# CommonRoad/commonroad-reactive-planner

Measured on AMD Instinct MI355X. Metric: candidate trajectories/sec (sample+cost+collision) per replan, higher is better.
Workload: dtype f64; 1 GPU; cfg3: DEU_Test-1_1_T-1, 31x31x63 grid, N=60, 51 obstacles (49 synthetic, seed 0); mode=draw, horizon_steps=60, n_obstacles=51, parallelism=one GPU, exchange=none

## Files before the change

commonroad-reactive-planner_amd/csrc/rp_host.hip:

```cpp
#include <hip/hip_runtime.h>
#include <hip/hip_ext.h>
#include <sched.h>

#include <algorithm>
#include <atomic>
#include <chrono>
#include <cmath>
#include <cstdio>
#include <cstdlib>
#include <cstring>
#include <mutex>
#include <new>
#include <string>
#include <unordered_map>
#include <vector>

#include "rp_kernels.h"
#include "rp_frontend.h"
#include "rp_corridor.h"
#include "rp_pool.h"
#include "rp_fold_static.h"
#include "rp_table_window.h"

namespace {
// ... 6 lines not shown
constexpr int kChunkMinWavesPerCU = 7;
constexpr int kCostMinPerCU = 832;
constexpr int kSweepMinPerCU = 512;
constexpr int kLazyCap[RP_LAZY_LEVELS] = {1024, 4096, 16384};
constexpr int kLazyOff[RP_LAZY_LEVELS] = {0, 1024, 5120};
constexpr int kLazyListWords = 21504;
constexpr uint32_t kLazyTarget[RP_LAZY_LEVELS] = {128, 1024, 8192};

using ResultBlock = FinalizeOut;

struct Options {
    int lanes = 0;
    int eval_block = 0;
    int cost_kernel = -1;
    int chunk_kernel = -1;
    int lazy = -1;
    int sweep = -1;
    int fused_lon = 1;
    int fused_lon_blocks = -1;
    int auto_materialize = 1;
    int shard_policy = 1;
    int stage_out = 1, row_padding = 1, row_align = 0, tail_split = 1;
    int fixed_stride = 1;
    int table_window = 1;
    int lean_broad = 1;
    int fold_static = -1;
    int fold_threshold = kFoldThreshold;
    int lon_publish = 1, inline_grids = 1, event_bracket = 0, winner_lanes_as_batch = 0, zero_copy = 1, coeff_groups = 1;
    int winner_skip_query = 1;
    int lazy_trace = 0, print_stamps = 0, timing = 0;
    int wait_mode = RP_WAIT_SPIN;
};
struct OptionDesc {
    const char *key;
    int Options::*field;
    const char *env;
    bool env_negates;
    int lo, hi;
};
const OptionDesc kOptionTable[] = {
    {"lanes", &Options::lanes, "RP_AMD_G", false, 0, 64},
    {"eval_block", &Options::eval_block, "RP_AMD_EVAL_BLOCK", false, 0, 256},
    {"cost_kernel", &Options::cost_kernel, "RP_AMD_COST_KERNEL", false, -1, 1},
    {"chunk_kernel", &Options::chunk_kernel, "RP_AMD_CHUNK_KERNEL", false, -1, 1},
    {"lazy", &Options::lazy, "RP_AMD_LAZY", false, -1, 1},
    {"sweep", &Options::sweep, "RP_AMD_SWEEP", false, -1, 1},
    {"fused_lon", &Options::fused_lon, "RP_AMD_NO_FUSED_LON", true, 0, 1},
    {"fused_lon_blocks", &Options::fused_lon_blocks, "RP_AMD_FUSED_LON_BLOCKS", false, -1, 1 << 20},
    {"auto_materialize", &Options::auto_materialize, "RP_AMD_NO_AUTO_MATERIALIZE", true, 0, 1},
    {"shard_policy", &Options::shard_policy, "RP_AMD_SHARD_POLICY", false, 0, 1},
    {"stage_out", &Options::stage_out, "RP_AMD_NO_STAGE_OUT", true, 0, 1},
    {"row_padding", &Options::row_padding, "RP_AMD_NO_ROW_PADDING", true, 0, 1},
    {"row_align", &Options::row_align, "RP_AMD_ROW_ALIGN", false, 0, 16},
    {"tail_split", &Options::tail_split, "RP_AMD_NO_TAIL_SPLIT", true, 0, 1},
    {"fixed_stride", &Options::fixed_stride, "RP_AMD_NO_FIXED_STRIDE", true, 0, 1},
    {"table_window", &Options::table_window, "RP_AMD_NO_TABLE_WINDOW", true, 0, 1},
    {"lean_broad", &Options::lean_broad, "RP_AMD_NO_LEAN_BROAD", true, 0, 1},
    {"fold_static", &Options::fold_static, "RP_AMD_FOLD_STATIC", false, -1, 1},
    {"fold_threshold", &Options::fold_threshold, "RP_AMD_FOLD_THRESHOLD", false, 1, 1 << 30},
    {"lon_publish", &Options::lon_publish, "RP_AMD_NO_LON_PUBLISH", true, 0, 1},
    {"inline_grids", &Options::inline_grids, "RP_AMD_NO_INLINE_GRIDS", true, 0, 1},
    {"event_bracket", &Options::event_bracket, "RP_AMD_EVENT_BRACKET", false, 0, 1},
    {"winner_lanes_as_batch", &Options::winner_lanes_as_batch, "RP_AMD_WINNER_G_AS_BATCH", false, 0, 1},
    {"winner_skip_query", &Options::winner_skip_query, "RP_AMD_NO_WINNER_SKIP_QUERY", true, 0, 1},
    {"zero_copy", &Options::zero_copy, "RP_AMD_NO_ZERO_COPY", true, 0, 1},
    {"coeff_groups", &Options::coeff_groups, "RP_AMD_NO_COEFF_GROUPS", true, 0, 1},
    {"lazy_trace", &Options::lazy_trace, "RP_AMD_LAZY_TRACE", false, 0, 1},
    {"print_stamps", &Options::print_stamps, "RP_AMD_PRINT_STAMPS", false, 0, 1},
    {"timing", &Options::timing, "RP_AMD_TIMING", false, 0, 1},
    {"wait_mode", &Options::wait_mode, "RP_AMD_WAIT_MODE", false, RP_WAIT_SPIN, RP_WAIT_EVENT},
};
const OptionDesc *find_option(const char *key) {
    if (!key) return nullptr;
    for (const OptionDesc &d : kOptionTable)
        if (std::strcmp(d.key, key) == 0) return &d;
    return nullptr;
}
void options_from_environment(Options &o) {
    for (const OptionDesc &d : kOptionTable) {
        const char *e = d.env ? std::getenv(d.env) : nullptr;
        if (!e) continue;
        const int v = d.env_negates ? 0 : std::atoi(e);
        if (v >= d.lo && v <= d.hi) o.*(d.field) = v;
    }
}

}

struct rp_ctx {
    Options opt;
    int device = 0;
    hipStream_t stream = nullptr;
    std::string err;
    int num_cus = 256;
    int profiling = 0;
    unsigned long long calls = 0;
    hipEvent_t ev0 = nullptr, ev1 = nullptr;
    bool time_next_launch = false, timed_by_launch = false;

    double *d_tables = nullptr;
    int n_ref = 0, search_iters = 0, n_buckets = 0, table_words = 0;
    double bucket_inv_h = 0.0;
    double proj_d_limit = 20.0;
    std::vector<double> h_pos;
    rpfe::Tables h_front;
    std::vector<double> cycle_buf;
// ... 21 lines not shown
    double *d_states = nullptr;
    double *d_compact = nullptr;
    size_t cap_compact = 0;
    size_t cap_states = 0;
    double *d_profile = nullptr, *d_profile_one = nullptr;
    size_t cap_profile = 0, cap_profile_one = 0;
    PairHdr *d_pair_hdr = nullptr, *d_pair_hdr_one = nullptr;
    size_t cap_pair_hdr = 0;
    void *d_partials = nullptr;
    int cap_partials = 0;
    unsigned long long *d_sel_scratch = nullptr;
    LazyCtl *d_lazy_ctl = nullptr;
    int32_t *d_lazy_lists = nullptr;
    uint32_t *d_lazy_hist = nullptr;
    double *d_lazy_states = nullptr;
    size_t cap_lazy_states = 0;
    int lazy_skip = 0, lazy_penalty = 0;
    int collision_mode = RP_COLLISION_AUTO;
    int last_kernel = 0;
    int last_fixed_stride = 0;
#ifdef RP_TIMELINE_LON
    int last_lon_grid = 0;
#endif
    int last_lon_lean = 0;
    int last_collision_level = 0;
    int last_lazy = 0;
    double last_best_cost = 0.0;
    int64_t last_best_index = -1;
    double path_us[2] = {0.0, 0.0};
    int path_n[2] = {0, 0};
    int path_since_probe = 0, path_regime = -1;
    bool path_adaptive = false;
    bool time_whole = false;
    std::chrono::steady_clock::time_point plan_t0;
    bool epilogue_dirty = false;
    struct Pending {
        bool active = false, cin = false, skip_eval = false, ticket = false, done = false, time_valid = false, mat = false, coeffs = false;
        unsigned long long seq = 0;
        int grid = 0;
        KArgs ka{};
        std::chrono::steady_clock::time_point tp0, tp1;
    } pending;
    struct LevelState {
        Pending pending;
        std::vector<char> staged;
        bool staged_on_device = false, last_rows_on_device = false;
// ... 142 lines not shown
int collision_level(const KArgs &ka) {
    if (!ka.has_obstacles || (ka.flags & RP_FLAG_SKIP_COLLISION)) return 0;
    return (ka.obs.n_sobb + ka.obs.n_tri + ka.obs.n_circ) > 0 ? 2 : 1;
}

const void *sweep_kernel_fn(bool cin, int coll, bool one_chunk) {
    if (cin) {
        if (coll == 2) return one_chunk ? (const void *)rp_eval_kernel<16, false, true, 2, true, false, false, RP_BLOCK, true> : (const void *)rp_eval_kernel<16, false, true, 2, false, false, false, RP_BLOCK, true>;
        return one_chunk ? (const void *)rp_eval_kernel<16, false, true, 1, true, false, false, RP_BLOCK, true> : (const void *)rp_eval_kernel<16, false, true, 1, false, false, false, RP_BLOCK, true>;
    }
    if (coll == 2) return one_chunk ? (const void *)rp_eval_kernel<16, false, false, 2, true, false, false, RP_BLOCK, true> : (const void *)rp_eval_kernel<16, false, false, 2, false, false, false, RP_BLOCK, true>;
    return one_chunk ? (const void *)rp_eval_kernel<16, false, false, 1, true, false, false, RP_BLOCK, true> : (const void *)rp_eval_kernel<16, false, false, 1, false, false, false, RP_BLOCK, true>;
}

const void *chunk_kernel_fn(bool low, int coll) {
    if (low) return coll == 2 ? (const void *)rp_chunk_kernel<true, 2> : (coll == 1 ? (const void *)rp_chunk_kernel<true, 1> : (const void *)rp_chunk_kernel<true, 0>);
    return coll == 2 ? (const void *)rp_chunk_kernel<false, 2> : (coll == 1 ? (const void *)rp_chunk_kernel<false, 1> : (const void *)rp_chunk_kernel<false, 0>);
}

inline bool fixed_stride_applies(const rp_ctx *c, const KArgs &ka) {
    return ka.row_stride == RP_ROW64 && ka.tail_split == 0 && ka.N + 1 > 16 && ka.N + 1 <= RP_ROW64 && c->opt.fixed_stride != 0;
}

template <int G, bool MAT, bool CIN, int COLL, bool STAGE>
void launch_eval_tcs(rp_ctx *c, const KArgs &ka, int grid, size_t lds, int block = RP_BLOCK) {
    if constexpr (G == 16 && MAT && !STAGE) {
        if (fixed_stride_applies(c, ka)) {
            if (block == 64) launch_kargs(c, (const void *)rp_eval_kernel<G, MAT, CIN, COLL, false, false, false, 64, false, true>, grid, 64, lds, ka);
            else launch_kargs(c, (const void *)rp_eval_kernel<G, MAT, CIN, COLL, false, false, false, RP_BLOCK, false, true>, grid, RP_BLOCK, lds, ka);
            return;
        }
    }
    if constexpr (G == 16 && !STAGE) {
        if (block == 64) {
            if (ka.N + 1 <= G) launch_kargs(c, (const void *)rp_eval_kernel<G, MAT, CIN, COLL, true, false, false, 64>, grid, 64, lds, ka);
            else launch_kargs(c, (const void *)rp_eval_kernel<G, MAT, CIN, COLL, false, false, false, 64>, grid, 64, lds, ka);
            return;
        }
    }
    if (ka.N + 1 <= G) launch_kargs(c, (const void *)rp_eval_kernel<G, MAT, CIN, COLL, true, STAGE, false>, grid, RP_BLOCK, lds, ka);
    else launch_kargs(c, (const void *)rp_eval_kernel<G, MAT, CIN, COLL, false, STAGE, false>, grid, RP_BLOCK, lds, ka);
}

constexpr int kFusedLonG = 16;
constexpr size_t kFusedLonLdsLimit = 61440;
int fused_lon_max_blocks(const rp_ctx *c) {
    if (c->opt.fused_lon_blocks >= 0) return c->opt.fused_lon_blocks;
    return c->num_cus * 4;
}

// ... 469 lines not shown
        const bool cost_rows_ok = (unsigned long long)ka.pair_count * PF_FIELDS * (unsigned long long)(ka.N + 1) * 8ull < (1ull << 32);
        const bool cost_big = count >= (int64_t)c->num_cus * 1024;
        auto lane_kernel_for = [&](int coll) -> int {
            if (!lane_kernel_ok) return 0;
            if (c->opt.chunk_kernel == 1 && chunk_G) return 2;
            if (!cost_rows_ok) return (chunk_G && c->opt.chunk_kernel != 0 && coll == 0) ? 2 : 0;
            if (c->opt.cost_kernel == 1) return 1;
            if (coll > 0) return (c->opt.cost_kernel != 0 && cost_big) ? 1 : 0;
            const int64_t chunk_waves = ((count + RP_CHUNK_BLOCK - 1) / RP_CHUNK_BLOCK) * chunk_G;
            const bool chunk_ok = c->opt.chunk_kernel != 0 && chunk_G && chunk_G <= 4 && chunk_waves >= (int64_t)c->num_cus * kChunkMinWavesPerCU;
            if (c->opt.cost_kernel != 0 && count >= (int64_t)c->num_cus * (chunk_ok ? kCostMinPerCU : (ka.N + 1 <= 64 ? 240 : 448))) return 1;
            return chunk_ok ? 2 : 0;
        };
        auto launch_main_eval = [&](const KArgs &k, bool mat_) -> int {
            c->timed_by_launch = false;
            c->time_next_launch = by_launch;
            if (timed && !by_launch) HIP_TRY(c, hipEventRecord(c->ev0, c->stream));
            const auto te0 = c->timing ? std::chrono::steady_clock::now() : std::chrono::steady_clock::time_point();
            const int coll = collision_level(k);
            const int which = mat_ ? 0 : lane_kernel_for(coll);
            if (which == 1) {
                main_grid = (int)((count + RP_COST_BLOCK - 1) / RP_COST_BLOCK);
                c->last_kernel = RP_KERNEL_COST;
                c->last_fixed_stride = 0;
                const void *fn = k.low_vel_mode
                    ? (coll == 2 ? (const void *)rp_cost_kernel<true, 2> : coll == 1 ? (const void *)rp_cost_kernel<true, 1> : (const void *)rp_cost_kernel<true, 0>)
                    : (coll == 2 ? (const void *)rp_cost_kernel<false, 2> : coll == 1 ? (const void *)rp_cost_kernel<false, 1> : (const void *)rp_cost_kernel<false, 0>);
                launch_kargs(c, fn, main_grid, RP_COST_BLOCK, 0, k);
            } else if (which == 2) {
                main_grid = (int)((count + RP_CHUNK_BLOCK - 1) / RP_CHUNK_BLOCK);
                c->last_kernel = RP_KERNEL_CHUNK;
                c->last_fixed_stride = 0;
                launch_kargs(c, chunk_kernel_fn(k.low_vel_mode != 0, coll), main_grid, RP_CHUNK_BLOCK * chunk_G, rp_chunk_lds_bytes(chunk_G), k);
            } else {
                main_grid = grid;
                c->last_kernel = RP_KERNEL_EVAL;
                c->last_fixed_stride = !fused_lds && mat_ && G == 16 && fixed_stride_applies(c, k);
                if (fused_lds) launch_eval_fused(c, k, grid, mat_, cin, fused_lds, G);
                else launch_eval(c, k, grid, mat_, cin, G, block);
            }
            if (c->timing) c->t_sum[4] += std::chrono::duration<double, std::micro>(std::chrono::steady_clock::now() - te0).count();
            c->time_next_launch = false;
            if (timed && !by_launch) HIP_TRY(c, hipEventRecord(c->ev1, c->stream));
            time_valid = timed && (!by_launch || c->timed_by_launch);
            return RP_OK;
        };
        bool lazy_possible = count > 0 && !mat && !fused_lds && collision_level(ka) > 0 && !(ka.flags & RP_FLAG_DRAW_ALL) &&
                             ka.cost_kind != RP_COST_EXTERNAL && !ka.single_index && !ka.gate;
        const int lazy_env = c->opt.lazy;
        lazy_possible = lazy_possible && lazy_env != 0 && (c->collision_mode != RP_COLLISION_EAGER || lazy_env == 1);
        const bool always = lazy_env == 1 || (lazy_env == -1 && c->collision_mode == RP_COLLISION_COST_ORDERED);
        bool lazy_try = lazy_possible && (always || (!small && c->lazy_skip == 0));
        if (lazy_possible && !lazy_try && !always && !small && c->lazy_skip > 0) --c->lazy_skip;
        c->path_adaptive = lazy_possible && lazy_env == -1 && !small && c->collision_mode == RP_COLLISION_TIMED;
        if (c->path_adaptive) {
            int lg = 0;
            while ((count >> (lg + 1)) != 0) ++lg;
            const int regime = 2 * lg + (cin ? 1 : 0);
            if (regime != c->path_regime) { c->path_regime = regime; c->path_n[0] = c->path_n[1] = 0; c->path_since_probe = 0; }
            if (lazy_try) {
// ... 335 lines not shown

int rp_last_path(const rp_ctx *c) { return c ? c->last_lazy : 0; }
int rp_last_kernel(const rp_ctx *c) { return c ? c->last_kernel : 0; }

int rp_set_collision_path(rp_ctx *c, int mode) {
    if (!c) return RP_EINVAL;
    if (mode < RP_COLLISION_AUTO || mode > RP_COLLISION_TIMED) return fail(c, RP_EINVAL, "rp_set_collision_path: unknown mode");
    if (mode != c->collision_mode) { c->lazy_skip = c->lazy_penalty = 0; c->path_regime = -1; }
    c->collision_mode = mode;
    return RP_OK;
}

int rp_set_profiling(rp_ctx *c, int enable) {
    if (!c) return RP_EINVAL;
    c->profiling = enable < 0 ? 0 : enable;
    return RP_OK;
}

int rp_set_option(rp_ctx *c, const char *key, int64_t value) {
    if (!c) return RP_EINVAL;
    if (c->pending.active) return fail(c, RP_ESTATE, "rp_set_option: a plan is in flight on this context (rp_plan_wait first)");
    const OptionDesc *d = find_option(key);
    if (!d) return fail(c, RP_EINVAL, std::string("rp_set_option: unknown option '") + (key ? key : "(null)") + "'");
    if (value < d->lo || value > d->hi) return fail(c, RP_EINVAL, std::string("rp_set_option: value out of range for '") + key + "'");
    c->opt.*(d->field) = (int)value;
    c->timing = c->opt.timing != 0;
    c->spin_wait = c->opt.wait_mode != RP_WAIT_EVENT;
    c->lazy_skip = c->lazy_penalty = 0; c->path_regime = -1;
    return RP_OK;
}

int rp_get_option(const rp_ctx *c, const char *key, int64_t *value) {
    if (!c || !value) return RP_EINVAL;
    if (key && std::strcmp(key, "wait_fallbacks") == 0) { *value = c->wait_fallbacks; return RP_OK; }
    if (key && std::strcmp(key, "last_fixed_stride") == 0) { *value = c->last_fixed_stride; return RP_OK; }
    if (key && std::strcmp(key, "last_lon_lean") == 0) { *value = c->last_lon_lean; return RP_OK; }
    if (key && std::strcmp(key, "last_collision_level") == 0) { *value = c->last_collision_level; return RP_OK; }
    if (key && std::strcmp(key, "fold_static_steps") == 0) { *value = c->d_fold ? c->fold_steps : 0; return RP_OK; }
    if (key && std::strcmp(key, "last_lanes") == 0) { *value = c->last_G; return RP_OK; }
    if (key && std::strcmp(key, "last_single_launch") == 0) { *value = c->last_fused_lds != 0 ? 1 : 0; return RP_OK; }
    if (key && std::strcmp(key, "last_table_window") == 0) { *value = c->have_last ? c->last.win_n : 0; return RP_OK; }
    if (key && std::strcmp(key, "last_table_window_first") == 0) { *value = c->have_last ? c->last.win_k0 : 0; return RP_OK; }
    const OptionDesc *d = find_option(key);
    if (!d) return RP_EINVAL;
    *value = c->opt.*(d->field);
    return RP_OK;
}

int rp_set_wait_mode(rp_ctx *c, int mode) { return rp_set_option(c, "wait_mode", mode); }
int rp_get_wait_mode(const rp_ctx *c) { return c ? c->opt.wait_mode : RP_WAIT_SPIN; }

int rp_set_reference(rp_ctx *c, int32_t n, const double *ref_pos, const double *ref_theta, const double *ref_curv,
                     const double *ref_curv_d, const double *ref_x, const double *ref_y, double proj_domain_d_limit) {
    if (!c) return RP_EINVAL;
    if (c->pending.active) return fail(c, RP_ESTATE, "rp_set_reference: a plan is in flight on this context (rp_plan_wait first)");
    if (n < 2 || !ref_pos || !ref_theta || !ref_curv || !ref_curv_d || !ref_x || !ref_y)
        return fail(c, RP_EINVAL, "rp_set_reference: need n >= 2 and six non-null tables");
    for (int i = 0; i + 1 < n; ++i)
// ... 1319 lines not shown
```

commonroad-reactive-planner_amd/csrc/rp_kernels.h:

```cpp
#pragma once

#include "rp_device.h"

#define RP_BLOCK 256
#ifndef RP_COPY_OUT_STORE
#define RP_COPY_OUT_STORE(p, v)                                                                                   \
    __builtin_nontemporal_store(*reinterpret_cast<const __attribute__((ext_vector_type(2))) double *>(&(v)),        \
                                reinterpret_cast<__attribute__((ext_vector_type(2))) double *>(p))
#endif
#ifndef RP_WAVES_PER_SIMD
#define RP_WAVES_PER_SIMD 3
#endif

struct KArgs {
    double dt;
    int32_t N, factor, time_step0, low_vel_mode, lon_mode;
    uint32_t constraint_mask, flags;
    double x0_lon[3], x0_lat[3], x0_orientation;
    double wheelbase, wb_rear_axle, half_length, half_width, ego_radius;
    double a_max, v_switch, v_delta_max, kappa_max;
    double c_yaw;
    double c_kdot;
    int32_t cost_kind, has_speed, has_s, partials_cap;
    double w_a, desired_speed, desired_d, desired_s;
// ... 899 lines not shown
    const bool fast = v > v_switch;
    const double acc_l = fast ? acc * v : acc, acc_r = fast ? a_max * v_switch : a_max;
    const bool bad_acc = !((-a_max <= acc) & (acc_l <= acc_r));
    const bool bad_v = v < -RP_EPS, bad_k = fabs(kappa) > kappa_max;
    reason = (((cm & RP_CHECK_ACCELERATION) != 0) & bad_acc) ? RP_REASON_ACCELERATION : reason;
    reason = (((cm & RP_CHECK_KAPPA_DOT) != 0) & bad_kd) ? RP_REASON_KAPPA_DOT : reason;
    reason = (((cm & RP_CHECK_YAW_RATE) != 0) & bad_yaw) ? RP_REASON_YAW_RATE : reason;
    reason = (((cm & RP_CHECK_KAPPA) != 0) & bad_k) ? RP_REASON_KAPPA : reason;
    reason = (((cm & RP_CHECK_VELOCITY) != 0) & bad_v) ? RP_REASON_VELOCITY : reason;
    return reason;
}

__device__ __forceinline__ void lateral_derivs(bool low, double dd, double ddd, double inv_sd, double sdd, double &dp, double &dpp) {
    if (!low) {
        dp = dd * inv_sd;
        const double ddot = ddd - dp * sdd;
        dpp = ddot * inv_sd * inv_sd;
    } else {
        dp = dd;
        dpp = ddd;
    }
}

__device__ __forceinline__ void atan_angles(double dp, double th_ref, double &th_cl, double &th_gl, double &cosT, double &secT, double &tanT) {
    th_cl = rp_atan(dp);
    th_gl = th_cl + th_ref;
    const double w2 = __builtin_fma(dp, dp, 1.0);
    cosT = rp_rsqrt(w2);
    secT = w2 * cosT;
    tanT = dp;
}

__device__ __forceinline__ void standstill_angles(double th_cl, bool use_atan, double &cosT, double &secT, double &tanT) {
    double sn, cs;
    rp_sincos(th_cl, &sn, &cs);
    const double sc = rp_rcp(cs);
    cosT = use_atan ? cosT : cs;
    secT = use_atan ? secT : sc;
    tanT = use_atan ? tanT : sn * sc;
}

__device__ __forceinline__ void frenet_kinematics(double d, double dp, double dpp, double sd, double sdd, double k_r, double k_r_d,
                                                  double cosT, double secT, double tanT, double &kappa, double &v, double &acc) {
    const double oneKrD = 1.0 - k_r * d;
    const double q = cosT * rp_rcp(oneKrD);
    const double kterm = frenet_kterm(k_r_d, d, k_r, dp);
    kappa = frenet_kappa(dpp, kterm, tanT, cosT, q, k_r);
    const double f = oneKrD * secT;
    v = sd * f;
    acc = frenet_acc(sdd, f, sd, secT, oneKrD, tanT, kappa, k_r, kterm);
}

__device__ __forceinline__ void extended_state(double l_v, double l_acc, double l_s, double l_sd, double l_d, double l_dd, double tk,
                                               double &vt, double &e_s, double &e_d) {
    vt = l_v + tk * l_acc;
    vt = vt * (vt >= 0.0 ? 1.0 : 0.0);
    e_s = l_s + tk * l_sd;
    e_d = l_d + tk * l_dd;
// ... 540 lines not shown
        pair = p32;
        ci.v[0] = grid_base(a)[a.nT + a.nL + (int)(g32 - p32 * nd)];
    }
    ci.pair_slot = pair - hdr_pair0;
}

__device__ __forceinline__ void fetch_header(const PairHdr *hdrs, CandIn &ci) {
    const PairHdr h = hdrs[ci.pair_slot];
    ci.lat_T = h.lat_T;
    ci.s0 = h.s0;
    ci.pre_reason = h.pre_reason;
    ci.L = h.L;
}

template <bool COEFFS_IN>
__device__ __forceinline__ CandIn fetch_candidate(const KArgs &a, int64_t gidx, const PairHdr *hdrs, int64_t hdr_pair0) {
    CandIn ci;
    fetch_lateral<COEFFS_IN>(a, gidx, ci, hdr_pair0);
    fetch_header(hdrs, ci);
    return ci;
}

#define RP_ROW64 64
template <int G, bool MAT, bool COEFFS_IN, int COLL, bool ONE_CHUNK, bool STAGE_OUT, bool LON_FUSED, int BLOCK = RP_BLOCK, bool SWEEP = false,
          bool ROW64 = false>
__global__ __launch_bounds__(BLOCK, RP_WAVES_PER_SIMD) void rp_eval_kernel(const KArgsG ag) {
    static_assert(!SWEEP || (G == 16 && !MAT && COLL != 0 && !STAGE_OUT && !LON_FUSED && BLOCK == RP_BLOCK), "the sweep's variant");
    static_assert(!ROW64 || (G == 16 && MAT && !ONE_CHUNK && !STAGE_OUT && !LON_FUSED && !SWEEP), "the fixed-stride variant");
    const KArgs &a = ag.k;
    extern __shared__ double lds_out[];
    static_assert(!(LON_FUSED && STAGE_OUT), "the single-launch variant stores state rows directly");
    constexpr bool RP_WT = LON_FUSED;
    constexpr bool RP_NT = MAT && !LON_FUSED && !STAGE_OUT;
    touch_kernargs<10>();

    const int tid = threadIdx.x;
    RP_STAMP(0);
    RP_TL(0);
    const int lane = tid & 63;
    const int gl = lane & (G - 1);
    const int gbase = lane & ~(G - 1);
    static_assert(BLOCK == RP_BLOCK || (!LON_FUSED && !STAGE_OUT), "smaller workgroups: plain two-kernel variants only");
    constexpr int GPB = BLOCK / G;
    constexpr int GPW = 64 / G;
    constexpr int PFN = COLL ? PF_FIELDS : PF_COS_REF;
    const int wave_in_block = tid >> 6;
    const int group_in_wave = gbase / G;
    const int grp = tid / G;

    if (level_gate_closed(a.gate, a.gate_seq, a.gate_level)) return;
    if (a.single_index && *a.single_index < 0) {
// ... 319 lines not shown
        if (al.has_s) { e = 0.25 * (al.desired_s - s); cst = __builtin_fma(e, e, cst); }
        if (i == N) {
            e = 20.0 * (al.desired_d - d); cst = __builtin_fma(e, e, cst);
            e = 5.0 * fabs(th_cl); cst = __builtin_fma(e, e, cst);
            if (al.has_speed) { e = v - al.desired_speed; cst += 50.0 * (e * e); }
            if (al.has_s) { e = 20.0 * (al.desired_s - s); cst = __builtin_fma(e, e, cst); }
        }
        if (i == mid && al.has_speed) { e = v - al.desired_speed; cst += 100.0 * (e * e); }
        return cst;
    };
    auto fetched_cost_terms = [&](const CostParams &cp, int i, double acc, double v, double s, double d, double th_cl) -> double {
        double e, cst;
        e = cp.w_a * acc; cst = e * e;
        e = 0.25 * (cp.desired_d - d); cst = __builtin_fma(e, e, cst);
        e = 0.25 * fabs(th_cl); cst = __builtin_fma(e, e, cst);
        if (cp.has_speed) { asm volatile(""); e = 5.0 * (v - cp.desired_speed); cst = __builtin_fma(e, e, cst); }
        if (cp.has_s) { asm volatile(""); e = 0.25 * (cp.desired_s - s); cst = __builtin_fma(e, e, cst); }
        if (i == N) {
            e = 20.0 * (cp.desired_d - d); cst = __builtin_fma(e, e, cst);
            e = 5.0 * fabs(th_cl); cst = __builtin_fma(e, e, cst);
            if (cp.has_speed) { asm volatile(""); e = v - cp.desired_speed; cst += 50.0 * (e * e); }
            if (cp.has_s) { asm volatile(""); e = 20.0 * (cp.desired_s - s); cst = __builtin_fma(e, e, cst); }
        }
        if (i == mid && cp.has_speed) { asm volatile(""); e = v - cp.desired_speed; cst += 100.0 * (e * e); }
        return cst;
    };

    if (wave_first < count) {
        const int64_t w0 = wave_first;
        const int64_t slot = w0 + group_in_wave;
        const bool valid = slot < count && sweep_need;
        const int64_t gidx = al.single_index ? *al.single_index
                             : ((!LON_FUSED && al.index_list) ? (int64_t)al.index_list[valid ? slot : w0] : al.cand_begin + (valid ? slot : w0));

        const int L = cin.L;
        const double s0 = cin.s0;
        const uint32_t pre_reason = (uint32_t)cin.pre_reason;
        const int32_t pair_slot_ = (int32_t)(pair_index<COEFFS_IN>(al, gidx) - pair0);
        const int32_t pair_w = __builtin_amdgcn_readfirstlane(pair_slot_);
        const uint32_t n8p = (uint32_t)n * 8u;
        const char *const pbase = reinterpret_cast<const char *>(prof_base + ((size_t)pair_w * PF_FIELDS) * (size_t)n);
        const uint32_t poff8 = (uint32_t)(pair_slot_ - pair_w) * PF_FIELDS * n8p;
        ProfStep pf = pf0;
        if (!LON_FUSED) {
            Poly lat;
            if (COEFFS_IN) lat = {cin.v[0], cin.v[1], cin.v[2], cin.v[3], cin.v[4], cin.v[5]};
            else lat = quintic_coeffs(al.x0_lat[0], al.x0_lat[1], al.x0_lat[2], cin.v[0], 0.0, 0.0, cin.lat_T);
// ... 53 lines not shown
                uint64_t near_sta_cell = 0;
                if (!SKIP_EXTENDED || __any(act)) {
                    const double t = (double)i * dt;
                    const double tau = low ? s - s0 : t;
                    d = poly_pos(gs_poly, tau); dd = poly_vel(gs_poly, tau); ddd = poly_acc(gs_poly, tau);
                    if (fabs(dd) < RP_EPS) dd = 0.0;
                    if (!LATE_STORE && store_ok && act) {
                        const uint32_t off8 = lane_off8 + (uint32_t)i * 8u;
                        st_row<RP_WT, RP_NT>(row_at(off8, RP_S), s);
                        st_row<RP_WT, RP_NT>(row_at(off8, RP_S_DOT), sd);
                        st_row<RP_WT, RP_NT>(row_at(off8, RP_S_DDOT), sdd);
                        st_row<RP_WT, RP_NT>(row_at(off8, RP_D), d);
                        st_row<RP_WT, RP_NT>(row_at(off8, RP_D_DOT), dd);
                        st_row<RP_WT, RP_NT>(row_at(off8, RP_D_DDOT), ddd);
                    }
                    RP_STAMP(3);

                    const bool moving = inv_sd > 0.0;
                    double dp, dpp;
                    lateral_derivs(low, dd, ddd, inv_sd, sdd, dp, dpp);

                    const bool use_atan = moving || low;
                    double cosT, secT, tanT;
                    atan_angles(dp, th_ref, th_cl, th_gl, cosT, secT, tanT);
                    if (__any(act && !use_atan)) {
                        const uint64_t mv = group_ballot<G>(use_atan && act, gbase);
                        const uint64_t below = mv & ((1ull << gl) - 1ull);
                        const int src = below ? 63 - __clzll(below) : 0;
                        const double th_from = group_bcast<G>(th_gl, src);
                        if (!use_atan) {
                            th_gl = below ? th_from : theta_carry;
                            th_cl = th_gl - th_ref;
                        }
                        standstill_angles(th_cl, use_atan, cosT, secT, tanT);
                    }
                    const double sinT = tanT * cosT;
                    cos_gl = heading_cos(pf.f[PF_COS_REF], pf.f[PF_SIN_REF], cosT, sinT);
                    sin_gl = heading_sin(pf.f[PF_COS_REF], pf.f[PF_SIN_REF], cosT, sinT);
                    RP_STAMP(5);

                    frenet_kinematics(d, dp, dpp, sd, sdd, k_r, k_r_d, cosT, secT, tanT, kappa, v, acc);

                    double th_prev = lane_prev(th_gl), ka_prev = lane_prev(kappa);
                    if (gl == 0) { th_prev = theta_carry; ka_prev = kappa_carry; }
                    const double dth = i > 0 ? th_gl - th_prev : 0.0;
                    kdot = i > 0 ? kappa - ka_prev : 0.0;
                    RP_STAMP(6);

                    uint32_t reason = constraint_reason(al, cm, v, acc, kappa, dth, kdot);
                    reason = act ? reason : RP_REASON_NONE;
                    if (__any(reason != RP_REASON_NONE)) {
                        const uint64_t fm = group_ballot<G>(reason != RP_REASON_NONE, gbase);
                        const int fl = fm ? __ffsll((unsigned long long)fm) - 1 : 0;
                        const uint32_t r_first = (uint32_t)__shfl((int)reason, fl, G);
                        if (fm && fail_step < 0) { fail_step = base + fl; fail_reason = r_first; }
                        if (!draw && fail_step >= 0) alive = false;
                        if (__ballot(alive) == 0) break;
                    }
                    RP_STAMP(7);

                    const bool in_dom = s_in_dom && fabs(d) <= al.proj_d_limit;
                    x = px + d * nx; y = py + d * ny;
                    if (__any(act && !in_dom) || ood_step >= 0) {
                        const uint64_t om = group_ballot<G>(act && !in_dom, gbase);
                        if (om && ood_step < 0) ood_step = base + __ffsll((unsigned long long)om) - 1;
                        if (ood_step >= 0 && i >= ood_step) { x = 0.0; y = 0.0; }
                    }
                    if (act) {
                        if (!LATE_STORE && store_ok) {
                            const uint32_t off8 = lane_off8 + (uint32_t)i * 8u;
                            st_row<RP_WT, RP_NT>(row_at(off8, RP_X), x);
                            st_row<RP_WT, RP_NT>(row_at(off8, RP_Y), y);
                            st_row<RP_WT, RP_NT>(row_at(off8, RP_THETA), th_gl);
                            st_row<RP_WT, RP_NT>(row_at(off8, RP_V), v);
                            st_row<RP_WT, RP_NT>(row_at(off8, RP_A), acc);
                            st_row<RP_WT, RP_NT>(row_at(off8, RP_KAPPA), kappa);
                            st_row<RP_WT, RP_NT>(row_at(off8, RP_KAPPA_DOT), kdot);
                            st_row<RP_WT, RP_NT>(row_at(off8, RP_THETA_CL), th_cl);
                        }
                        if (!LEAN) cost_acc += eval_cost_terms(i, acc, v, s, d, th_cl);
                    }
                    if (!LEAN && COLL == 2 && live && alive && fail_step < 0 && ood_step < 0 && !collide && act)
                        near_sta_cell = static_grid_mask(al.obs.grid, al.obs.gx0, al.obs.gy0, al.obs.ginv, al.obs.gnx, al.obs.gny,
                                                         x + al.wb_rear_axle * cos_gl, y + al.wb_rear_axle * sin_gl);
                }
                const bool cell_wanted = COLL == 2 && live && alive && fail_step < 0 && ood_step < 0 && !collide;
                RP_STAMP(8);

                const int ll = L - 1 - base;
                const bool take = (ll >= 0 && ll < G);
                if (__any(take && L < n)) {
                    if (!COLL) rp_sincos(th_gl, &sin_gl, &cos_gl);
                    if (take && gl == ll) {
                        double *o = gs_last;
                        o[0] = x; o[1] = y; o[2] = th_gl; o[3] = v; o[4] = acc; o[5] = kappa; o[6] = kdot;
                        o[7] = s; o[8] = d; o[9] = th_cl; o[10] = sd; o[11] = sdd; o[12] = dd; o[13] = ddd;
                        o[14] = cos_gl; o[15] = sin_gl;
                    }
                }
                if (!ONE_CHUNK && c + 1 < nchunks) {
                    theta_carry = group_bcast<G>(th_gl, G - 1);
                    kappa_carry = group_bcast<G>(kappa, G - 1);
                }
                if (__any(live && !act)) {
                    double termx = 0.0, termy = 0.0;
                    const double *o = gs_last;
                    const double tk = (double)(i - L + 1) * dt;
                    double vt = 0.0;
                    if (!act) {
                        vt = o[3] + tk * o[4];
                        vt = vt * (vt >= 0.0 ? 1.0 : 0.0);
                        termx = dt * vt * o[14];
                        termy = dt * vt * o[15];
                    }
                    const double scx = group_scan<G>(termx) + cumx, scy = group_scan<G>(termy) + cumy;
// ... 860 lines not shown
```

commonroad-reactive-planner_amd/csrc/rp_math.h:

```cpp
#pragma once

#include <hip/hip_runtime.h>

#ifndef RP_FMA3_ASM
#define RP_FMA3_ASM 1
#endif
__device__ __forceinline__ double rp_fma3(double a, double b, double c) {
#if RP_FMA3_ASM
    double r;
    asm("v_fma_f64 %0, %1, %2, %3" : "=v"(r) : "v"(a), "v"(b), "v"(c));
    return r;
#else
    return __builtin_fma(a, b, c);
#endif
}
__device__ __forceinline__ double rp_fma3_first(double x, double c1, double c0) {
#if RP_FMA3_ASM
    double r;
    asm("v_fma_f64 %0, %1, %2, %3" : "=v"(r) : "s"(c1), "v"(x), "v"(c0));
    return r;
#else
    return __builtin_fma(x, c1, c0);
#endif
}

__device__ __forceinline__ double rp_rcp(double x) {
    double y = __builtin_amdgcn_rcp(x);
    double e = __builtin_fma(-x, y, 1.0);
    y = __builtin_fma(y, e, y);
    e = __builtin_fma(-x, y, 1.0);
    return __builtin_fma(y, e, y);
}

__device__ __forceinline__ double rp_rsqrt(double x) {
    double y = __builtin_amdgcn_rsq(x);
    double r = x * y;
    double e = __builtin_fma(-r, y, 1.0);
    double t = __builtin_fma(0.375, e, 0.5);
    return __builtin_fma(y * e, t, y);
}

__device__ __forceinline__ double rp_atan_poly(double t) {
    const double z = t * t, w = z * z;
    double s1 = rp_fma3_first(w, 1.62858201153657823623e-02, 4.97687799461593236017e-02);
    s1 = rp_fma3(w, s1, 6.66107313738753120669e-02);
    s1 = rp_fma3(w, s1, 9.09088713343650656196e-02);
    s1 = rp_fma3(w, s1, 1.42857142725034663711e-01);
    s1 = rp_fma3(w, s1, 3.33333333333329318027e-01);
    s1 = z * s1;
    double s2 = rp_fma3_first(w, -3.65315727442169155270e-02, -5.83357013379057348645e-02);
    s2 = rp_fma3(w, s2, -7.69187620504482999495e-02);
    s2 = rp_fma3(w, s2, -1.11111104054623557880e-01);
    s2 = rp_fma3(w, s2, -1.99999999998764832476e-01);
    s2 = w * s2;
    return t * (s1 + s2);
}

__device__ __forceinline__ double rp_atan(double x) {
    const double ax = fabs(x);
    const bool r0 = ax < 0.4375;
    double t = ax, hi = 0.0, lo = 0.0;
    if (!__all(r0)) {
        const bool r1 = ax < 0.6875, r2 = ax < 1.1875, r3 = ax < 2.4375;
        const double num = r0 ? ax : (r1 ? __builtin_fma(2.0, ax, -1.0) : (r2 ? ax - 1.0 : (r3 ? ax - 1.5 : -1.0)));
        const double den = r0 ? 1.0 : (r1 ? 2.0 + ax : (r2 ? ax + 1.0 : (r3 ? __builtin_fma(1.5, ax, 1.0) : ax)));
        t = r0 ? num : num * rp_rcp(den);
        hi = r0 ? 0.0 : (r1 ? 4.63647609000806093515e-01 : (r2 ? 7.85398163397448278999e-01
                : (r3 ? 9.82793723247329054082e-01 : 1.57079632679489655800e+00)));
        lo = r0 ? 0.0 : (r1 ? 2.26987774529616870924e-17 : (r2 ? 3.06161699786838301793e-17
                : (r3 ? 1.39033110312309984516e-17 : 6.12323399573676603587e-17)));
        if (ax > 7.3786976294838206464e19) t = 0.0;
    }
    const double p = rp_atan_poly(t);
    const double res = hi - ((p - lo) - t);
    return copysign(res, x);
}

__device__ __forceinline__ void rp_sincos(double x, double *s, double *c) {
    const double n = rint(x * 6.36619772367581382433e-01);
    double r = __builtin_fma(-n, 1.57079632673412561417e+00, x);
    const double y = __builtin_fma(-n, 6.07710050650619224932e-11, r);
    const double z = y * y;
    double ps = rp_fma3_first(z, 1.58969099521155010221e-10, -2.50507602534068634195e-08);
    ps = rp_fma3(z, ps, 2.75573137070700676789e-06);
    ps = rp_fma3(z, ps, -1.98412698298579493134e-04);
    ps = rp_fma3(z, ps, 8.33333333332248946124e-03);
    ps = rp_fma3(z, ps, -1.66666666666666324348e-01);
    const double sn = __builtin_fma(y * z, ps, y);
    double pc = rp_fma3_first(z, -1.13596475577881948265e-11, 2.08757232129817482790e-09);
    pc = rp_fma3(z, pc, -2.75573143513906633035e-07);
    pc = rp_fma3(z, pc, 2.48015872894767294178e-05);
    pc = rp_fma3(z, pc, -1.38888888888741095749e-03);
    pc = rp_fma3(z, pc, 4.16666666666666019037e-02);
    const double hz = 0.5 * z;
    const double w1 = 1.0 - hz;
    const double cs = w1 + (((1.0 - w1) - hz) + z * z * pc);
    const int q = (int)n & 3;
    const double ss = (q & 1) ? cs : sn;
    const double cc = (q & 1) ? sn : cs;
    *s = (q & 2) ? -ss : ss;
    *c = ((q + 1) & 2) ? -cc : cc;
}

__device__ __forceinline__ double ext_travel(double v, double acc, int m, double dt) {
    const double h = dt * acc;
    double t0 = 1.0, t1 = (double)m;
    if (h < 0.0) {
        if (!(v > 0.0)) return 0.0;
        t1 = fmin(t1, floor(v * rp_rcp(-h)));
    } else if (v < 0.0) {
        if (!(h > 0.0)) return 0.0;
        t0 = fmax(t0, floor(-v * rp_rcp(h)) + 1.0);
    }
    if (t1 < t0) return 0.0;
    const double cnt = t1 - t0 + 1.0;
    return dt * (cnt * v + h * 0.5 * (t0 + t1) * cnt);
// ... 3 lines not shown
```

Measured before the change: 474.3 million candidates/s.

## Add four-waves-per-SIMD fixed-stride eval variant with register-light math constants

Adds a W4 instance of the fixed-stride eval kernel whose launch bounds ask for four waves per SIMD, and selects it by default through a new eval_waves option. To fit the tighter VGPR budget, polynomial constants in atan and sincos are materialised in SGPRs or right at use instead of being kept live in vector registers. The midpoint index is recomputed in a scalar register, and the first-lane search uses 32-bit ffs. The aim is higher occupancy to hide f64 latency, at the risk of register spills or extra instructions in the hot loop.

Measured after the change: 504.3 million candidates/s (median of 6 runs). 6.3% higher.

```diff
diff --git a/commonroad-reactive-planner_amd/csrc/rp_host.hip b/commonroad-reactive-planner_amd/csrc/rp_host.hip
--- a/commonroad-reactive-planner_amd/csrc/rp_host.hip
+++ b/commonroad-reactive-planner_amd/csrc/rp_host.hip
@@ -52,6 +52,7 @@
     int shard_policy = 1;
     int stage_out = 1, row_padding = 1, row_align = 0, tail_split = 1;
     int fixed_stride = 1;
+    int eval_waves = 0;
     int table_window = 1;
     int lean_broad = 1;
     int fold_static = -1;
@@ -84,6 +85,7 @@
     {"row_align", &Options::row_align, "RP_AMD_ROW_ALIGN", false, 0, 16},
     {"tail_split", &Options::tail_split, "RP_AMD_NO_TAIL_SPLIT", true, 0, 1},
     {"fixed_stride", &Options::fixed_stride, "RP_AMD_NO_FIXED_STRIDE", true, 0, 1},
+    {"eval_waves", &Options::eval_waves, "RP_AMD_EVAL_WAVES", false, 0, 4},
     {"table_window", &Options::table_window, "RP_AMD_NO_TABLE_WINDOW", true, 0, 1},
     {"lean_broad", &Options::lean_broad, "RP_AMD_NO_LEAN_BROAD", true, 0, 1},
     {"fold_static", &Options::fold_static, "RP_AMD_FOLD_STATIC", false, -1, 1},
@@ -106,12 +108,16 @@
         if (std::strcmp(d.key, key) == 0) return &d;
     return nullptr;
 }
+bool option_value_ok(const OptionDesc &d, int64_t v) {
+    if (v < d.lo || v > d.hi) return false;
+    return d.field != &Options::eval_waves || v == 0 || v >= 3;
+}
 void options_from_environment(Options &o) {
     for (const OptionDesc &d : kOptionTable) {
         const char *e = d.env ? std::getenv(d.env) : nullptr;
         if (!e) continue;
         const int v = d.env_negates ? 0 : std::atoi(e);
-        if (v >= d.lo && v <= d.hi) o.*(d.field) = v;
+        if (option_value_ok(d, v)) o.*(d.field) = v;
     }
 }
 
@@ -179,6 +185,7 @@
 #ifdef RP_TIMELINE_LON
     int last_lon_grid = 0;
 #endif
+    int last_eval_waves = 0;
     int last_lon_lean = 0;
     int last_collision_level = 0;
     int last_lazy = 0;
@@ -367,10 +374,17 @@
     return ka.row_stride == RP_ROW64 && ka.tail_split == 0 && ka.N + 1 > 16 && ka.N + 1 <= RP_ROW64 && c->opt.fixed_stride != 0;
 }
 
+inline int eval_waves_for(const rp_ctx *c) { return c->opt.eval_waves != 0 ? c->opt.eval_waves : 4; }
+
 template <int G, bool MAT, bool CIN, int COLL, bool STAGE>
 void launch_eval_tcs(rp_ctx *c, const KArgs &ka, int grid, size_t lds, int block = RP_BLOCK) {
     if constexpr (G == 16 && MAT && !STAGE) {
         if (fixed_stride_applies(c, ka)) {
+            if (eval_waves_for(c) == 4) {
+                if (block == 64) launch_kargs(c, (const void *)rp_eval_kernel<G, MAT, CIN, COLL, false, false, false, 64, false, true, true>, grid, 64, lds, ka);
+                else launch_kargs(c, (const void *)rp_eval_kernel<G, MAT, CIN, COLL, false, false, false, RP_BLOCK, false, true, true>, grid, RP_BLOCK, lds, ka);
+                return;
+            }
             if (block == 64) launch_kargs(c, (const void *)rp_eval_kernel<G, MAT, CIN, COLL, false, false, false, 64, false, true>, grid, 64, lds, ka);
             else launch_kargs(c, (const void *)rp_eval_kernel<G, MAT, CIN, COLL, false, false, false, RP_BLOCK, false, true>, grid, RP_BLOCK, lds, ka);
             return;
@@ -886,7 +900,7 @@
             if (which == 1) {
                 main_grid = (int)((count + RP_COST_BLOCK - 1) / RP_COST_BLOCK);
                 c->last_kernel = RP_KERNEL_COST;
-                c->last_fixed_stride = 0;
+                c->last_fixed_stride = c->last_eval_waves = 0;
                 const void *fn = k.low_vel_mode
                     ? (coll == 2 ? (const void *)rp_cost_kernel<true, 2> : coll == 1 ? (const void *)rp_cost_kernel<true, 1> : (const void *)rp_cost_kernel<true, 0>)
                     : (coll == 2 ? (const void *)rp_cost_kernel<false, 2> : coll == 1 ? (const void *)rp_cost_kernel<false, 1> : (const void *)rp_cost_kernel<false, 0>);
@@ -894,12 +908,13 @@
             } else if (which == 2) {
                 main_grid = (int)((count + RP_CHUNK_BLOCK - 1) / RP_CHUNK_BLOCK);
                 c->last_kernel = RP_KERNEL_CHUNK;
-                c->last_fixed_stride = 0;
+                c->last_fixed_stride = c->last_eval_waves = 0;
                 launch_kargs(c, chunk_kernel_fn(k.low_vel_mode != 0, coll), main_grid, RP_CHUNK_BLOCK * chunk_G, rp_chunk_lds_bytes(chunk_G), k);
             } else {
                 main_grid = grid;
                 c->last_kernel = RP_KERNEL_EVAL;
                 c->last_fixed_stride = !fused_lds && mat_ && G == 16 && fixed_stride_applies(c, k);
+                c->last_eval_waves = c->last_fixed_stride ? eval_waves_for(c) : 3;
                 if (fused_lds) launch_eval_fused(c, k, grid, mat_, cin, fused_lds, G);
                 else launch_eval(c, k, grid, mat_, cin, G, block);
             }
@@ -1281,7 +1296,7 @@
     if (c->pending.active) return fail(c, RP_ESTATE, "rp_set_option: a plan is in flight on this context (rp_plan_wait first)");
     const OptionDesc *d = find_option(key);
     if (!d) return fail(c, RP_EINVAL, std::string("rp_set_option: unknown option '") + (key ? key : "(null)") + "'");
-    if (value < d->lo || value > d->hi) return fail(c, RP_EINVAL, std::string("rp_set_option: value out of range for '") + key + "'");
+    if (!option_value_ok(*d, value)) return fail(c, RP_EINVAL, std::string("rp_set_option: value out of range for '") + key + "'");
     c->opt.*(d->field) = (int)value;
     c->timing = c->opt.timing != 0;
     c->spin_wait = c->opt.wait_mode != RP_WAIT_EVENT;
@@ -1293,6 +1308,7 @@
     if (!c || !value) return RP_EINVAL;
     if (key && std::strcmp(key, "wait_fallbacks") == 0) { *value = c->wait_fallbacks; return RP_OK; }
     if (key && std::strcmp(key, "last_fixed_stride") == 0) { *value = c->last_fixed_stride; return RP_OK; }
+    if (key && std::strcmp(key, "last_eval_waves") == 0) { *value = c->last_eval_waves; return RP_OK; }
     if (key && std::strcmp(key, "last_lon_lean") == 0) { *value = c->last_lon_lean; return RP_OK; }
     if (key && std::strcmp(key, "last_collision_level") == 0) { *value = c->last_collision_level; return RP_OK; }
     if (key && std::strcmp(key, "fold_static_steps") == 0) { *value = c->d_fold ? c->fold_steps : 0; return RP_OK; }
diff --git a/commonroad-reactive-planner_amd/csrc/rp_kernels.h b/commonroad-reactive-planner_amd/csrc/rp_kernels.h
--- a/commonroad-reactive-planner_amd/csrc/rp_kernels.h
+++ b/commonroad-reactive-planner_amd/csrc/rp_kernels.h
@@ -945,8 +945,9 @@
     }
 }
 
+template <bool SC = false>
 __device__ __forceinline__ void atan_angles(double dp, double th_ref, double &th_cl, double &th_gl, double &cosT, double &secT, double &tanT) {
-    th_cl = rp_atan(dp);
+    th_cl = rp_atan<SC>(dp);
     th_gl = th_cl + th_ref;
     const double w2 = __builtin_fma(dp, dp, 1.0);
     cosT = rp_rsqrt(w2);
@@ -954,9 +955,10 @@
     tanT = dp;
 }
 
+template <bool SC = false>
 __device__ __forceinline__ void standstill_angles(double th_cl, bool use_atan, double &cosT, double &secT, double &tanT) {
     double sn, cs;
-    rp_sincos(th_cl, &sn, &cs);
+    rp_sincos<SC>(th_cl, &sn, &cs);
     const double sc = rp_rcp(cs);
     cosT = use_atan ? cosT : cs;
     secT = use_atan ? secT : sc;
@@ -1543,11 +1545,14 @@
 }
 
 #define RP_ROW64 64
+template <bool NARROW>
+__device__ __forceinline__ int group_first(uint64_t m) { return NARROW ? __ffs((int)(uint32_t)m) - 1 : __ffsll((unsigned long long)m) - 1; }
 template <int G, bool MAT, bool COEFFS_IN, int COLL, bool ONE_CHUNK, bool STAGE_OUT, bool LON_FUSED, int BLOCK = RP_BLOCK, bool SWEEP = false,
-          bool ROW64 = false>
-__global__ __launch_bounds__(BLOCK, RP_WAVES_PER_SIMD) void rp_eval_kernel(const KArgsG ag) {
+          bool ROW64 = false, bool W4 = false>
+__global__ __launch_bounds__(BLOCK, W4 ? 4 : RP_WAVES_PER_SIMD) void rp_eval_kernel(const KArgsG ag) {
     static_assert(!SWEEP || (G == 16 && !MAT && COLL != 0 && !STAGE_OUT && !LON_FUSED && BLOCK == RP_BLOCK), "the sweep's variant");
     static_assert(!ROW64 || (G == 16 && MAT && !ONE_CHUNK && !STAGE_OUT && !LON_FUSED && !SWEEP), "the fixed-stride variant");
+    static_assert(!W4 || ROW64, "four wavefronts per SIMD: an instance of the fixed-stride variant only");
     const KArgs &a = ag.k;
     extern __shared__ double lds_out[];
     static_assert(!(LON_FUSED && STAGE_OUT), "the single-launch variant stores state rows directly");
@@ -1913,7 +1918,9 @@
             if (cp.has_speed) { asm volatile(""); e = v - cp.desired_speed; cst += 50.0 * (e * e); }
             if (cp.has_s) { asm volatile(""); e = 20.0 * (cp.desired_s - s); cst = __builtin_fma(e, e, cst); }
         }
-        if (i == mid && cp.has_speed) { asm volatile(""); e = v - cp.desired_speed; cst += 100.0 * (e * e); }
+        int mid_l = mid;
+        if (W4) { int nn = N; asm volatile("" : "+s"(nn)); mid_l = (nn + 1) / 2; }
+        if (i == mid_l && cp.has_speed) { asm volatile(""); e = v - cp.desired_speed; cst += 100.0 * (e * e); }
         return cst;
     };
 
@@ -2013,7 +2020,7 @@
 
                     const bool use_atan = moving || low;
                     double cosT, secT, tanT;
-                    atan_angles(dp, th_ref, th_cl, th_gl, cosT, secT, tanT);
+                    atan_angles<W4>(dp, th_ref, th_cl, th_gl, cosT, secT, tanT);
                     if (__any(act && !use_atan)) {
                         const uint64_t mv = group_ballot<G>(use_atan && act, gbase);
                         const uint64_t below = mv & ((1ull << gl) - 1ull);
@@ -2023,7 +2030,7 @@
                             th_gl = below ? th_from : theta_carry;
                             th_cl = th_gl - th_ref;
                         }
-                        standstill_angles(th_cl, use_atan, cosT, secT, tanT);
+                        standstill_angles<W4>(th_cl, use_atan, cosT, secT, tanT);
                     }
                     const double sinT = tanT * cosT;
                     cos_gl = heading_cos(pf.f[PF_COS_REF], pf.f[PF_SIN_REF], cosT, sinT);
@@ -2042,7 +2049,7 @@
                     reason = act ? reason : RP_REASON_NONE;
                     if (__any(reason != RP_REASON_NONE)) {
                         const uint64_t fm = group_ballot<G>(reason != RP_REASON_NONE, gbase);
-                        const int fl = fm ? __ffsll((unsigned long long)fm) - 1 : 0;
+                        const int fl = fm ? group_first<W4>(fm) : 0;
                         const uint32_t r_first = (uint32_t)__shfl((int)reason, fl, G);
                         if (fm && fail_step < 0) { fail_step = base + fl; fail_reason = r_first; }
                         if (!draw && fail_step >= 0) alive = false;
@@ -2054,7 +2061,7 @@
                     x = px + d * nx; y = py + d * ny;
                     if (__any(act && !in_dom) || ood_step >= 0) {
                         const uint64_t om = group_ballot<G>(act && !in_dom, gbase);
-                        if (om && ood_step < 0) ood_step = base + __ffsll((unsigned long long)om) - 1;
+                        if (om && ood_step < 0) ood_step = base + group_first<W4>(om);
                         if (ood_step >= 0 && i >= ood_step) { x = 0.0; y = 0.0; }
                     }
                     if (act) {
@@ -2081,7 +2088,7 @@
                 const int ll = L - 1 - base;
                 const bool take = (ll >= 0 && ll < G);
                 if (__any(take && L < n)) {
-                    if (!COLL) rp_sincos(th_gl, &sin_gl, &cos_gl);
+                    if (!COLL) rp_sincos<W4>(th_gl, &sin_gl, &cos_gl);
                     if (take && gl == ll) {
                         double *o = gs_last;
                         o[0] = x; o[1] = y; o[2] = th_gl; o[3] = v; o[4] = acc; o[5] = kappa; o[6] = kdot;
diff --git a/commonroad-reactive-planner_amd/csrc/rp_math.h b/commonroad-reactive-planner_amd/csrc/rp_math.h
--- a/commonroad-reactive-planner_amd/csrc/rp_math.h
+++ b/commonroad-reactive-planner_amd/csrc/rp_math.h
@@ -24,6 +24,43 @@
 #endif
 }
 
+__device__ __forceinline__ double rp_scalar_here(double c) {
+    uint32_t lo, hi;
+    asm volatile("s_mov_b32 %0, %1" : "=s"(lo) : "i"((uint32_t)__builtin_bit_cast(uint64_t, c)));
+    asm volatile("s_mov_b32 %0, %1" : "=s"(hi) : "i"((uint32_t)(__builtin_bit_cast(uint64_t, c) >> 32)));
+    return __builtin_bit_cast(double, ((uint64_t)hi << 32) | lo);
+}
+__device__ __forceinline__ double rp_vector_here(double c) {
+    uint32_t lo, hi;
+    asm volatile("v_mov_b32 %0, %1" : "=v"(lo) : "i"((uint32_t)__builtin_bit_cast(uint64_t, c)));
+    asm volatile("v_mov_b32 %0, %1" : "=v"(hi) : "i"((uint32_t)(__builtin_bit_cast(uint64_t, c) >> 32)));
+    return __builtin_bit_cast(double, ((uint64_t)hi << 32) | lo);
+}
+template <bool SC>
+__device__ __forceinline__ double rp_select_const(double c) { return SC ? rp_vector_here(c) : c; }
+__device__ __forceinline__ double rp_fma3_sc(double a, double b, double c) {
+#if RP_FMA3_ASM
+    double r;
+    asm("v_fma_f64 %0, %1, %2, %3" : "=v"(r) : "v"(a), "v"(b), "s"(rp_scalar_here(c)));
+    return r;
+#else
+    return __builtin_fma(a, b, c);
+#endif
+}
+__device__ __forceinline__ double rp_fma3_first_sc(double x, double c1, double c0) {
+#if RP_FMA3_ASM
+    double r;
+    asm("v_mov_b64 %0, %1\n\tv_fmac_f64 %0, %2, %3" : "=&v"(r) : "s"(rp_scalar_here(c0)), "s"(rp_scalar_here(c1)), "v"(x));
+    return r;
+#else
+    return __builtin_fma(x, c1, c0);
+#endif
+}
+template <bool SC>
+__device__ __forceinline__ double rp_fma3_by(double a, double b, double c) { return SC ? rp_fma3_sc(a, b, c) : rp_fma3(a, b, c); }
+template <bool SC>
+__device__ __forceinline__ double rp_fma3_first_by(double x, double c1, double c0) { return SC ? rp_fma3_first_sc(x, c1, c0) : rp_fma3_first(x, c1, c0); }
+
 __device__ __forceinline__ double rp_rcp(double x) {
     double y = __builtin_amdgcn_rcp(x);
     double e = __builtin_fma(-x, y, 1.0);
@@ -40,22 +77,24 @@
     return __builtin_fma(y * e, t, y);
 }
 
+template <bool SC = false>
 __device__ __forceinline__ double rp_atan_poly(double t) {
     const double z = t * t, w = z * z;
-    double s1 = rp_fma3_first(w, 1.62858201153657823623e-02, 4.97687799461593236017e-02);
-    s1 = rp_fma3(w, s1, 6.66107313738753120669e-02);
-    s1 = rp_fma3(w, s1, 9.09088713343650656196e-02);
-    s1 = rp_fma3(w, s1, 1.42857142725034663711e-01);
-    s1 = rp_fma3(w, s1, 3.33333333333329318027e-01);
+    double s1 = rp_fma3_first_by<SC>(w, 1.62858201153657823623e-02, 4.97687799461593236017e-02);
+    s1 = rp_fma3_by<SC>(w, s1, 6.66107313738753120669e-02);
+    s1 = rp_fma3_by<SC>(w, s1, 9.09088713343650656196e-02);
+    s1 = rp_fma3_by<SC>(w, s1, 1.42857142725034663711e-01);
+    s1 = rp_fma3_by<SC>(w, s1, 3.33333333333329318027e-01);
     s1 = z * s1;
-    double s2 = rp_fma3_first(w, -3.65315727442169155270e-02, -5.83357013379057348645e-02);
-    s2 = rp_fma3(w, s2, -7.69187620504482999495e-02);
-    s2 = rp_fma3(w, s2, -1.11111104054623557880e-01);
-    s2 = rp_fma3(w, s2, -1.99999999998764832476e-01);
+    double s2 = rp_fma3_first_by<SC>(w, -3.65315727442169155270e-02, -5.83357013379057348645e-02);
+    s2 = rp_fma3_by<SC>(w, s2, -7.69187620504482999495e-02);
+    s2 = rp_fma3_by<SC>(w, s2, -1.11111104054623557880e-01);
+    s2 = rp_fma3_by<SC>(w, s2, -1.99999999998764832476e-01);
     s2 = w * s2;
     return t * (s1 + s2);
 }
 
+template <bool SC = false>
 __device__ __forceinline__ double rp_atan(double x) {
     const double ax = fabs(x);
     const bool r0 = ax < 0.4375;
@@ -65,33 +104,34 @@
         const double num = r0 ? ax : (r1 ? __builtin_fma(2.0, ax, -1.0) : (r2 ? ax - 1.0 : (r3 ? ax - 1.5 : -1.0)));
         const double den = r0 ? 1.0 : (r1 ? 2.0 + ax : (r2 ? ax + 1.0 : (r3 ? __builtin_fma(1.5, ax, 1.0) : ax)));
         t = r0 ? num : num * rp_rcp(den);
-        hi = r0 ? 0.0 : (r1 ? 4.63647609000806093515e-01 : (r2 ? 7.85398163397448278999e-01
-                : (r3 ? 9.82793723247329054082e-01 : 1.57079632679489655800e+00)));
-        lo = r0 ? 0.0 : (r1 ? 2.26987774529616870924e-17 : (r2 ? 3.06161699786838301793e-17
-                : (r3 ? 1.39033110312309984516e-17 : 6.12323399573676603587e-17)));
+        hi = r0 ? 0.0 : (r1 ? rp_select_const<SC>(4.63647609000806093515e-01) : (r2 ? rp_select_const<SC>(7.85398163397448278999e-01)
+                : (r3 ? rp_select_const<SC>(9.82793723247329054082e-01) : rp_select_const<SC>(1.57079632679489655800e+00))));
+        lo = r0 ? 0.0 : (r1 ? rp_select_const<SC>(2.26987774529616870924e-17) : (r2 ? rp_select_const<SC>(3.06161699786838301793e-17)
+                : (r3 ? rp_select_const<SC>(1.39033110312309984516e-17) : rp_select_const<SC>(6.12323399573676603587e-17))));
         if (ax > 7.3786976294838206464e19) t = 0.0;
     }
-    const double p = rp_atan_poly(t);
+    const double p = rp_atan_poly<SC>(t);
     const double res = hi - ((p - lo) - t);
     return copysign(res, x);
 }
 
+template <bool SC = false>
 __device__ __forceinline__ void rp_sincos(double x, double *s, double *c) {
     const double n = rint(x * 6.36619772367581382433e-01);
     double r = __builtin_fma(-n, 1.57079632673412561417e+00, x);
     const double y = __builtin_fma(-n, 6.07710050650619224932e-11, r);
     const double z = y * y;
-    double ps = rp_fma3_first(z, 1.58969099521155010221e-10, -2.50507602534068634195e-08);
-    ps = rp_fma3(z, ps, 2.75573137070700676789e-06);
-    ps = rp_fma3(z, ps, -1.98412698298579493134e-04);
-    ps = rp_fma3(z, ps, 8.33333333332248946124e-03);
-    ps = rp_fma3(z, ps, -1.66666666666666324348e-01);
+    double ps = rp_fma3_first_by<SC>(z, 1.58969099521155010221e-10, -2.50507602534068634195e-08);
+    ps = rp_fma3_by<SC>(z, ps, 2.75573137070700676789e-06);
+    ps = rp_fma3_by<SC>(z, ps, -1.98412698298579493134e-04);
+    ps = rp_fma3_by<SC>(z, ps, 8.33333333332248946124e-03);
+    ps = rp_fma3_by<SC>(z, ps, -1.66666666666666324348e-01);
     const double sn = __builtin_fma(y * z, ps, y);
-    double pc = rp_fma3_first(z, -1.13596475577881948265e-11, 2.08757232129817482790e-09);
-    pc = rp_fma3(z, pc, -2.75573143513906633035e-07);
-    pc = rp_fma3(z, pc, 2.48015872894767294178e-05);
-    pc = rp_fma3(z, pc, -1.38888888888741095749e-03);
-    pc = rp_fma3(z, pc, 4.16666666666666019037e-02);
+    double pc = rp_fma3_first_by<SC>(z, -1.13596475577881948265e-11, 2.08757232129817482790e-09);
+    pc = rp_fma3_by<SC>(z, pc, -2.75573143513906633035e-07);
+    pc = rp_fma3_by<SC>(z, pc, 2.48015872894767294178e-05);
+    pc = rp_fma3_by<SC>(z, pc, -1.38888888888741095749e-03);
+    pc = rp_fma3_by<SC>(z, pc, 4.16666666666666019037e-02);
     const double hz = 0.5 * z;
     const double w1 = 1.0 - hz;
     const double cs = w1 + (((1.0 - w1) - hz) + z * z * pc);
```
